# geopolars/geopolars

Measured on AMD Instinct MI355X. Metric: predicate evals/sec (10M pts x 1k polys point-in-polygon), higher is better.
Workload: dtype f64

## Files before the change

geopolars_amd/csrc/gpk_join.hip:

```cpp
#include <cstdlib>
#include <cstring>
#include <mutex>
#include <type_traits>

#include <rocprim/rocprim.hpp>

#include "gpk_device.h"
#include "gpk_index.h"
#include "gpk_candjoin.h"
#include "gpk_pip.h"
#include "gpk_scan.h"
#include "gpk_pipshared.h"

namespace gpk {

constexpr int PIP_BLOCK = 256;
constexpr int WR_BLOCK = 256;
constexpr int PIP_PPT = 2;
constexpr int PIP_TILE = PIP_BLOCK * PIP_PPT;
constexpr int PIP_GS = 8;
constexpr int PIP_OVF = 256;
constexpr int PIP_QCAP = PIP_BLOCK * PIP_PPT;
constexpr int PIP_SUPER_SHIFT = 6;
constexpr int PIP_WPT = 8;
// ... 1151 lines not shown
    for (int k = 0; k < PIP_WPT; ++k) {
        if (cnt[k] == 0) continue;
        const uint32_t l = left_base + (uint32_t)(i0 + k);
        if (c[k] != CODE_MULTI && (c[k] & CODE_POOL)) {
            const uint32_t at = c[k] & ~CODE_POOL;
            for (uint32_t t = 0; t < cnt[k]; ++t) emit(o++, make_uint2(l, multi_pool[at + 1 + t]));
            continue;
        }
        if (c[k] != CODE_MULTI) {
            emit(o++, make_uint2(l, c[k]));
            continue;
        }
        const double2 p = pts.xy[i0 + k];
        const GridParams g = *ix.grid;
        for_each_candidate(ix, g, p.x, p.y, [&](int j) {
            if (dev::valid_row(polys.validity, j) && dev::polygonal_hits_point<false>(polys, j, p.x, p.y)) emit(o++, make_uint2(l, (uint32_t)j));
        });
    }
    if (via_lds) {
        __syncthreads();
        const int n_out = (int)tot;
        for (int t = tid; t < n_out; t += WR_BLOCK)
            if (out_base + t < capacity) pairs[out_base + t] = s_pairs[t];
    }
}

constexpr size_t JOIN_STATS_WORDS = 8 + 8 * 8000;
static unsigned long long* g_join_stats = nullptr;
static bool g_join_stats_on = false;
unsigned long long* join_stats_buffer() { return g_join_stats_on ? g_join_stats : nullptr; }

static std::mutex g_fused_mu;
struct FusedDev {
    unsigned long long* slots = nullptr;
    unsigned long long tickets = 0;
    unsigned long long era = 0;
    int n = 0;
    hipEvent_t done = nullptr;
    hipStream_t last = nullptr;
    bool any = false;
};
static FusedDev g_fused[16];
static unsigned long long g_fused_epoch = 0;
struct FusedWords {
    unsigned long long *slots, *ticket, *lost;
    unsigned long long epoch, ticket_base;
};
static int32_t fused_launch_begin(hipStream_t s, int64_t n_words, int wgs, FusedWords* out) {
    int dev = 0;
    GPK_HIP(hipGetDevice(&dev));
    if (dev < 0 || dev >= 16) return fail(GPK_ERR_DEVICE, "spatial_join: device %d out of range", dev);
    if (n_words > (int64_t)0x7FFFFFF0ll) return fail(GPK_ERR_INVALID_ARGUMENT, "spatial_join: %lld epoch words", (long long)n_words);
    g_fused_mu.lock();
    FusedDev& f = g_fused[dev];
    auto bail = [&](hipError_t e) {
        g_fused_mu.unlock();
        return fail(GPK_ERR_DEVICE, "spatial_join: %s", hipGetErrorString(e));
    };
    if ((int64_t)f.n < n_words) {
        if (f.slots) {
            (void)hipDeviceSynchronize();
            (void)hipFree(f.slots);
            f.slots = nullptr;
        }
        const int want = n_words < 4096 ? 4096 : (int)n_words;
        const size_t bytes = sizeof(unsigned long long) * (size_t)(want + 2);
        hipError_t e = device_malloc((void**)&f.slots, bytes);
        if (e != hipSuccess) return bail(e);
        e = hipMemset(f.slots, 0, bytes);
        if (e != hipSuccess) return bail(e);
        f.n = want;
        f.tickets = 0;
        f.era = g_fused_epoch >> (64 - FUSED_TOTAL_BITS);
    }
    if (!f.done) {
        const hipError_t e = hipEventCreateWithFlags(&f.done, hipEventDisableTiming);
        if (e != hipSuccess) return bail(e);
    }
    if (f.any && f.last != s) {
        hipError_t e = hipEventRecord(f.done, f.last);
        if (e == hipSuccess) e = hipStreamWaitEvent(s, f.done, 0);
        if (e != hipSuccess) {
            (void)hipGetLastError();
            e = hipDeviceSynchronize();
            if (e != hipSuccess) return bail(e);
        }
    }
    ++g_fused_epoch;
    if ((g_fused_epoch & ((1ull << (64 - FUSED_TOTAL_BITS)) - 1ull)) == 0ull) ++g_fused_epoch;
    if ((g_fused_epoch >> (64 - FUSED_TOTAL_BITS)) != f.era) {
        const hipError_t e = hipMemsetAsync(f.slots, 0, sizeof(unsigned long long) * (size_t)(f.n + 1), s);
        if (e != hipSuccess) return bail(e);
        f.era = g_fused_epoch >> (64 - FUSED_TOTAL_BITS);
    }
    out->epoch = g_fused_epoch & ((1ull << (64 - FUSED_TOTAL_BITS)) - 1ull);
    out->slots = f.slots;
    out->lost = f.slots + f.n;
    out->ticket = f.slots + f.n + 1;
    out->ticket_base = f.tickets;
    f.tickets += (unsigned long long)wgs;
    return GPK_OK;
}
static void fused_launch_end(hipStream_t s, bool launched) {
    int dev = 0;
    (void)hipGetDevice(&dev);
    if (dev >= 0 && dev < 16) {
        g_fused[dev].last = s;
        g_fused[dev].any = true;
        if (!launched) g_fused[dev].n = 0;
    }
    g_fused_mu.unlock();
}

static int32_t pip_join_enqueue(const gpk_geoarray* left, const gpk_geoarray* right, const gpk_index* right_index, uint32_t left_row_base,
                                uint32_t* out_counts, uint32_t* out_pairs, int64_t pair_capacity, bool host_out,
                                unsigned long long* total_out, hipStream_t s, uint32_t** counts_dev_out, uint32_t** pairs_dev_out,
                                unsigned long long** grand_out) {
    const int64_t n = left->d.n_geoms;
    const bool lean = right_index->pip.R > 0 && right_index->pip_lean;
    static const bool no_flow = [] {
        const char* e = getenv("GPK_TILE_KERNEL");
        return e && !strcmp(e, "chain");
    }();
    PipView pvj = right_index->pip;
    pvj.slab_xy = right->d.xy;
    const bool chain = right_index->pip.R > 0 && right_index->pip.chain_xy != nullptr;
    const bool one_per_lane = !chain && !lean && right_index->pip.R > 0 && right_index->pip_list_heavy;
    const int flow_p = chain && !no_flow && right_index->pip.route != nullptr && right_index->pip.R <= PIP_ROUTE_RMAX
                           ? pip_flow_points_per_lane(n, right->d.n_geoms, right_index->pip.R, cu_count())
                           : 0;
    const bool flow = flow_p > 0;
    const int tile_points = flow ? 64 * flow_p : (chain ? 64 * CHAIN_PPT : (lean ? LEAN_TILE : (one_per_lane ? PIP_BLOCK : PIP_TILE)));
    const int64_t n_blocks = (n + tile_points - 1) / tile_points;
    const bool want_pairs = pair_capacity > 0;
    const size_t counts_bytes = sizeof(uint32_t) * (size_t)n;
    const size_t pairs_bytes = sizeof(uint32_t) * 2 * (size_t)pair_capacity;
    const int64_t n_super = (n_blocks >> PIP_SUPER_SHIFT) + 1;
    const int64_t n_wblocks = (n + PIP_WTILE - 1) / PIP_WTILE;
    const uint32_t multi_cap = chain ? 1024u : (uint32_t)(n < (int64_t)0x18000000 ? 2 * n + 1024 : (int64_t)0x30000000);
    int64_t flow_wgs = (int64_t)cu_count();
    {
        const int64_t want = (n_blocks + 15) / 16;
// ... 54 lines not shown
        hot.logR = 0;
        while ((1 << hot.logR) < pv.R) ++hot.logR;
        hot.rx0 = pv.rx0;
        hot.ry0 = pv.ry0;
        hot.inv_fw = pv.inv_fw;
        hot.inv_fh = pv.inv_fh;
        hot.cell = pv.cell;
        hot.half = reinterpret_cast<const HalfCell*>(pv.sub);
        hot.chain_xy = pv.chain_xy;
        hot.part_geom = pv.part_geom;
        hot.route = pv.route;
        hot.counts = counts_dev;
        hot.code = code;
        hot.block_tot = btot;
        hot.super_tot = stot;
        hot.stats = stats;
        hot.cold = cold;
        hot.stage = nullptr;
        hot.pool = reinterpret_cast<uint32_t*>(stage);
        hot.n_full_tiles = left->d.validity ? 0 : (int32_t)(n / tile_points);
        hot.inv_fw_s = pv.inv_fw * (double)PIP_SUB;
        hot.inv_fh_s = pv.inv_fh * (double)PIP_SUB;
        hot.sub_max = (double)(((uint32_t)PIP_SUB << hot.logR) - 1u);
    }
    if (flow) {
        const int64_t wgs = flow_wgs;
        FusedTail tail;
        memset(&tail, 0, sizeof tail);
        tail.pairs = (uint2*)pairs_dev;
        tail.capacity = pair_capacity;
        tail.grand = grand;
        tail.grand_host = total_out;
        tail.left_base = left_row_base;
        FusedWords fw;
        int32_t frc = fused_launch_begin(s, wgs, (int)wgs, &fw);
        if (frc != GPK_OK) return frc;
        tail.slots = fw.slots;
        tail.epoch = fw.epoch;
        tail.ticket = fw.ticket;
        tail.ticket_base = fw.ticket_base;
        tail.lost = fw.lost;
        frc = launch_pip_flow(hot, tail, (int)wgs, flow_p, s);
        fused_launch_end(s, frc == GPK_OK);
        if (frc != GPK_OK) return frc;
        *counts_dev_out = counts_dev;
        *pairs_dev_out = pairs_dev;
        *grand_out = grand;
        return GPK_OK;
    }
    if (chain)
        GPK_LAUNCH("gpk_pip_tile", pip_tile_chain_kernel, dim3((unsigned)((n_blocks + PIP_BLOCK / 64 - 1) / (PIP_BLOCK / 64))), dim3(PIP_BLOCK), 0, s, hot);
    else if (lean)
        GPK_LAUNCH("gpk_pip_tile", pip_tile_lean_kernel, dim3((unsigned)n_blocks), dim3(PIP_BLOCK), 0, s, left->d, right->d, right_index->v, pvj,
                 counts_dev, code, btot, stot, stats);
    else if (right_index->pip.R > 0)
        if (right_index->pip.sub2 && one_per_lane)
            GPK_LAUNCH("gpk_pip_tile", (pip_tile_kernel<true, true, 1>), dim3((unsigned)n_blocks), dim3(PIP_BLOCK), 0, s, left->d, right->d,
                     right_index->v, pvj, counts_dev, code, btot, stot, multi_pool, multi_cap, multi_top, stats);
        else if (right_index->pip.sub2)
            GPK_LAUNCH("gpk_pip_tile", (pip_tile_kernel<true, true>), dim3((unsigned)n_blocks), dim3(PIP_BLOCK), 0, s, left->d, right->d,
                     right_index->v, pvj, counts_dev, code, btot, stot, multi_pool, multi_cap, multi_top, stats);
        else if (one_per_lane)
            GPK_LAUNCH("gpk_pip_tile", (pip_tile_kernel<true, false, 1>), dim3((unsigned)n_blocks), dim3(PIP_BLOCK), 0, s, left->d, right->d,
                     right_index->v, pvj, counts_dev, code, btot, stot, multi_pool, multi_cap, multi_top, stats);
        else
            GPK_LAUNCH("gpk_pip_tile", (pip_tile_kernel<true, false>), dim3((unsigned)n_blocks), dim3(PIP_BLOCK), 0, s, left->d, right->d,
                     right_index->v, pvj, counts_dev, code, btot, stot, multi_pool, multi_cap, multi_top, stats);
    else
        GPK_LAUNCH("gpk_pip_tile_generic", (pip_tile_kernel<false, false>), dim3((unsigned)n_blocks), dim3(PIP_BLOCK), 0, s, left->d, right->d,
                 right_index->v, pvj, counts_dev, code, btot, stot, multi_pool, multi_cap, multi_top, stats);
    GPK_LAUNCH("gpk_pip_write", pip_write_kernel, dim3((unsigned)n_wblocks), dim3(WR_BLOCK), 0, s, left->d, right->d, right_index->v,
             code, btot, stot, (const uint32_t*)multi_pool, n_blocks, tile_points, left_row_base, (uint2*)pairs_dev, pair_capacity, grand, total_out);

    *counts_dev_out = counts_dev;
// ... 239 lines not shown
```

geopolars_amd/csrc/gpk_pipflow.hip:

```cpp
#include "gpk_pipshared.h"

namespace gpk {

constexpr int FLOW_P_MAX = 8;
constexpr int FLOW_BLOCK = 1024, FLOW_W = FLOW_BLOCK / 64;
constexpr int FLOW_ITEMS = 128;
constexpr int FLOW_PASS_AT = 40;
constexpr int FLOW_MAX_TILES = 1536;
constexpr int FLOW_ID_BITS = 22;
constexpr uint32_t FLOW_DEAD = 0xFFFFFFFFu;
constexpr uint32_t FLOW_MULTI = 0x80000000u;
constexpr uint32_t FLOW_PEND = FLOW_MULTI;
static_assert(64 * FLOW_P_MAX == 512, "an entry keeps the row within its tile in 9 bits");
static_assert(FLOW_MAX_TILES <= (1 << 14), "FlowItem::loc keeps the tile in 14 bits");

struct FlowItem {
    double px, py;
    uint32_t aux;
    uint32_t loc;
};
static_assert(sizeof(FlowItem) == 24, "list slot");

#ifdef GPK_TILE_TRACE
#define FLOW_STAMP(i)                                                                                                    \
    do {                                                                                                                 \
        if (h.stats && lane == 0 && wave % 5 == 0 && blockIdx.x < 900u) h.stats[8 + (blockIdx.x * 4 + wave / 5) * 16 + (i)] = wall_clock64(); \
    } while (0)
#if GPK_TILE_TRACE == 2
#define FLOW_PHASE(i)                                        \
    do {                                                     \
        asm volatile("s_waitcnt vmcnt(0) lgkmcnt(0)" ::: "memory"); \
        const unsigned long long _n = wall_clock64();        \
        g_phase[i] += _n - g_last;                           \
        g_last = _n;                                         \
    } while (0)
#define FLOW_PHASE_ARGS , unsigned long long (&g_phase)[6], unsigned long long& g_last
#define FLOW_PHASE_PASS , g_phase, g_last
#else
#define FLOW_PHASE(i) do {} while (0)
#define FLOW_PHASE_ARGS
#define FLOW_PHASE_PASS
#endif
#else
#define FLOW_STAMP(i) do {} while (0)
#define FLOW_PHASE(i) do {} while (0)
// ... 17 lines not shown
}

__device__ __forceinline__ void ring_edge_flat(double sx, double sy, double ex, double ey, double cx, double cy, int& wn, bool& on, bool& unsure) {
    const bool up = sy <= cy && ey >= cy, down = sy > cy && ey <= cy;
    const bool left = cx < fmin(sx, ex), within = !left && cx <= fmax(sx, ex);
    const double detleft = (sx - cx) * (ey - cy), detright = (sy - cy) * (ex - cx);
    const double det = detleft - detright;
    const double errbound = 3.3306690738754716e-16 * (fabs(detleft) + fabs(detright));
    const bool opposite = (detleft > 0.0 && detright <= 0.0) || (detleft < 0.0 && detright >= 0.0) || detleft == 0.0;
    const bool certain = opposite || fabs(det) >= errbound;
    const bool eval = (up || down) && within;
    unsure |= eval && !certain;
    on |= eval && certain && det == 0.0;
    wn += (up && ey != cy && (left || (within && det > 0.0))) ? 1 : 0;
    wn -= (down && (left || (within && det < 0.0))) ? 1 : 0;
}

__device__ __forceinline__ void flow_settle(const ChainHot& h, uint32_t* s_ttot, uint32_t t, uint32_t slot, uint32_t row, uint32_t li, uint32_t cnt,
                                            uint32_t first) {
    if (cnt == 0u) {
        h.pool[slot] = FLOW_DEAD;
        if (h.counts) h.counts[row] = 0u;
        atomicSub(&s_ttot[t], 1u);
    } else if (cnt == 1u) {
        h.pool[slot] = (first << 9) | li;
    } else {
        h.pool[slot] = FLOW_MULTI | (cnt << 9) | li;
        if (h.counts) h.counts[row] = cnt;
        atomicAdd(&s_ttot[t], cnt - 1u);
    }
}

template <int TS>
__device__ __forceinline__ void flow_exact_pass(const ChainHot& h, FlowItem* items, uint32_t& n_list, int lane, uint32_t* s_ttot, uint32_t tile0) {
    const uint32_t n = n_list < 64u ? n_list : 64u;
    wave_lds_fence();
    const bool act = (uint32_t)lane < n;
    double qx = 0.0, qy = 0.0;
    uint32_t hd = 0u, loc = 0u;
    if (act) {
        const FlowItem* it = items + lane;
        qx = it->px;
        qy = it->py;
        hd = it->aux;
        loc = it->loc;
    }
    const int count = (int)(hd & HCHAIN_COUNT_MASK);
    const double2* __restrict__ v = H_COLD(chain_xy) + (hd >> HCHAIN_START_SHIFT);
    const int i1 = count < 1 ? count : 1, i2 = count < 2 ? count : 2, i3 = count < 3 ? count : 3, i4 = count < 4 ? count : 4;
    double2 a0 = v[0], a1 = v[i1], a2 = v[i2], a3 = v[i3], a4 = v[i4];
    asm volatile("" : "+v"(a0.x), "+v"(a0.y), "+v"(a1.x), "+v"(a1.y), "+v"(a2.x), "+v"(a2.y), "+v"(a3.x), "+v"(a3.y), "+v"(a4.x), "+v"(a4.y));
    int wn = ((int)(hd << (28 - HCHAIN_BASE_SHIFT))) >> 28;
    bool unsure = false, on = false;
    ring_edge_flat(a0.x, a0.y, a1.x, a1.y, qx, qy, wn, on, unsure);
    ring_edge_flat(a1.x, a1.y, a2.x, a2.y, qx, qy, wn, on, unsure);
    ring_edge_flat(a2.x, a2.y, a3.x, a3.y, qx, qy, wn, on, unsure);
    ring_edge_flat(a3.x, a3.y, a4.x, a4.y, qx, qy, wn, on, unsure);
    if (count > 4) {
        double ax = a4.x, ay = a4.y;
        for (int j = 4; j < count; ++j) {
            const double2 b = v[j + 1];
            on |= dev::ring_edge_filtered(ax, ay, b.x, b.y, qx, qy, wn, unsure);
            ax = b.x;
            ay = b.y;
        }
    }
    const bool walk = act && (count == 0 || unsure);
    const bool inside = !on && wn != 0;
    const uint32_t t = loc >> 18, li = loc & 511u;
    const uint32_t slot = ((tile0 + t) << TS) + ((loc >> 9) & 511u), row = ((tile0 + t) << TS) + li;
    if (act && !walk && !inside) flow_settle(h, s_ttot, t, slot, row, li, 0u, 0u);
    unsigned long long wm = __ballot(walk);
#ifdef GPK_TILE_TRACE
    unsigned long long* const stats = nullptr;
#else
    unsigned long long* const stats = H_COLD(stats);
#endif
    if (stats) {
        const unsigned long long edges = wave_sum_u64((unsigned long long)(act ? count : 0));
        if (lane == 0) {
            atomicAdd(&stats[0], (unsigned long long)n);
            atomicAdd(&stats[1], edges);
            if (wm) atomicAdd(&stats[2], (unsigned long long)__popcll(wm));
        }
    }
    while (wm) {
        const int j = __builtin_ctzll(wm);
        wm &= wm - 1ull;
        const double x = __shfl(qx, j, 64), y = __shfl(qy, j, 64);
        const unsigned long long cf = chain_generic_row_first_call(H_COLD(cold), x, y, lane);
        if (lane == j) flow_settle(h, s_ttot, t, slot, row, li, (uint32_t)cf, (uint32_t)(cf >> 32));
    }
    n_list -= n;
    if (n_list) {
        FlowItem keep{};
        if ((uint32_t)lane < n_list) keep = items[64 + lane];
        wave_lds_fence();
        if ((uint32_t)lane < n_list) items[lane] = keep;
    }
    wave_lds_fence();
}

typedef uint32_t u32x4 __attribute__((ext_vector_type(4)));
// ... 2 lines not shown
                                                        uint32_t* s_ttot, uint32_t t, uint32_t tile, uint32_t n_ent, int lane, int ts) {
    asm volatile("s_waitcnt vmcnt(0)" ::: "memory");
    uint32_t* seg = pool + ((size_t)tile << ts);
    for (uint32_t i = 0; i < n_ent; i += 64u) {
        const uint32_t e = i + (uint32_t)lane < n_ent ? __hip_atomic_load(seg + i + lane, __ATOMIC_RELAXED, __HIP_MEMORY_SCOPE_AGENT) : 0u;
        unsigned long long pm = __ballot((e & ~511u) == FLOW_PEND);
        while (pm) {
            const int j = __builtin_ctzll(pm);
            pm &= pm - 1ull;
            const uint32_t li = (uint32_t)__shfl((int)e, j, 64) & 511u, row = (tile << ts) + li, slot = i + (uint32_t)j;
            const double2 q = pts_xy[row];
            const unsigned long long cf = chain_generic_row_first_call(cold, q.x, q.y, lane);
            const uint32_t cnt = (uint32_t)cf, first = (uint32_t)(cf >> 32);
            if (lane == 0) {
                if (stats) atomicAdd(&stats[2], 1ull);
                if (cnt == 0u) {
                    seg[slot] = FLOW_DEAD;
                    if (counts) counts[row] = 0u;
                    atomicSub(&s_ttot[t], 1u);
                } else if (cnt == 1u) {
                    seg[slot] = (first << 9) | li;
                } else {
                    seg[slot] = FLOW_MULTI | (cnt << 9) | li;
                    if (counts) counts[row] = cnt;
                    atomicAdd(&s_ttot[t], cnt - 1u);
                }
            }
        }
    }
}

template <bool SIMPLE, bool FULL, int P>
__device__ __forceinline__ void flow_tile(const ChainHot& h, const uint2* s_mask, const uint32_t* s_rec0, FlowItem* items, uint32_t& n_list, uint32_t t,
                                          uint32_t tile0, int lane, uint32_t* s_tcand, uint32_t* s_ttot FLOW_PHASE_ARGS) {
    constexpr int S = PIP_SUB, FLOW_TILE = 64 * P, TS = P == 8 ? 9 : (P == 4 ? 8 : (P == 2 ? 7 : 6));
    static_assert(P == 1 || P == 2 || P == 4 || P == 8, "tile sizes");
    static_assert(S == 8, "the sub-cell arithmetic below is written for 8 x 8 sub-cells");
    asm volatile("" : "+v"(lane));
    const uint32_t tile = tile0 + t;
    const int64_t base = (int64_t)tile * FLOW_TILE;
    const int64_t n_points = FULL ? 0 : H_COLD(n_points);
    const uint32_t rem = FULL ? (uint32_t)FLOW_TILE : (uint32_t)(n_points - base < (int64_t)FLOW_TILE ? n_points - base : (int64_t)FLOW_TILE);
    double px[P], py[P];
    {
        const double2* __restrict__ tile_xy = h.pts_xy + base;
        static_for<P>([&](auto K) {
            constexpr int k = decltype(K)::value;
            double2 v = make_double2(NAN, NAN);
            if (FULL || ((uint32_t)(k * 64 + lane) < rem && dev::valid_row(H_COLD(pts_validity), base + k * 64 + lane))) v = dev::load_stream(tile_xy + (k * 64 + lane));
            px[k] = v.x;
            py[k] = v.y;
        });
    }
    GPK_SCHED_FENCE();
    FLOW_PHASE(1);
    const int logR = h.logR;
    const uint32_t sub_max = ((uint32_t)S << logR) - 1u;
    uint32_t sidx4[(P + 3) / 4], gw[P];
    u32x4 rec[P];
    static_for<(P + 3) / 4>([&](auto J) { sidx4[decltype(J)::value] = 0u; });
    uint32_t sxs[P], sys_[P], r0s[P];
    uint2 ms[P];
    static_for<P>([&](auto K) {
        constexpr int k = decltype(K)::value;
        uint32_t sx = cvt_u32_sat((px[k] - h.rx0) * h.inv_fw_s), sy = cvt_u32_sat((py[k] - h.ry0) * h.inv_fh_s);
        sx = sx < sub_max ? sx : sub_max;
        sy = sy < sub_max ? sy : sub_max;
        const uint32_t at = ((sy >> 3) << (logR - 5)) + (sx >> 8);
        ms[k] = s_mask[at];
        r0s[k] = s_rec0[at];
        sxs[k] = sx;
        sys_[k] = sy;
// ... 82 lines not shown
    const bool live = e != FLOW_DEAD;
    const bool multi = live && (e & FLOW_MULTI) != 0u;
    const unsigned long long mm = __ballot(multi);
    if (__builtin_expect(mm == 0ull, 1)) {
        const unsigned long long m = __ballot(live);
        const uint32_t at = done + lanes_below(m);
        if (live && at < room) __builtin_nontemporal_store(((unsigned long long)(e >> 9) << 32) | (unsigned long long)(row0 + (e & 511u)), out64 + at);
        done += (uint32_t)__popcll(m);
        return;
    }
    const uint32_t n_out = !live ? 0u : (multi ? (e >> 9) & ((1u << FLOW_ID_BITS) - 1u) : 1u);
    uint32_t incl = n_out;
#pragma unroll
    for (int o = 1; o < 64; o <<= 1) {
        const uint32_t v = __shfl_up(incl, o, 64);
        if (lane >= o) incl += v;
    }
    const uint32_t at = done + incl - n_out;
    if (live && !multi && at < room) __builtin_nontemporal_store(((unsigned long long)(e >> 9) << 32) | (unsigned long long)(row0 + (e & 511u)), out64 + at);
    unsigned long long wm = mm;
    while (wm) {
        const int j = __builtin_ctzll(wm);
        wm &= wm - 1ull;
        const uint32_t lj = (uint32_t)__shfl((int)e, j, 64) & 511u, aj = (uint32_t)__shfl((int)at, j, 64);
        const double2 q = h.pts_xy[pt0 + lj];
        chain_generic_row_call(H_COLD(cold), q.x, q.y, lane, reinterpret_cast<uint2*>(out64 + aj), aj < room ? room - aj : 0u, row0 + lj);
    }
    done += (uint32_t)__shfl((int)incl, 63, 64);
}

template <bool SIMPLE, int P>
__global__ __launch_bounds__(FLOW_BLOCK) void pip_tile_flow_kernel(ChainHot h, FusedTail tail) {
    constexpr int WORDS = PIP_ROUTE_RMAX * PIP_ROUTE_RMAX / 32, W = FLOW_W, TS = P == 8 ? 9 : (P == 4 ? 8 : (P == 2 ? 7 : 6));
    __shared__ uint2 s_mask[WORDS];
    __shared__ uint32_t s_rec0[WORDS];
    __shared__ FlowItem s_items[W][FLOW_ITEMS];
    __shared__ uint32_t s_tcand[FLOW_MAX_TILES], s_ttot[FLOW_MAX_TILES];
    __shared__ uint32_t s_next, s_next2, s_wg, s_wgtot, s_gave_up;
    __shared__ unsigned long long s_part[W];
    const int lane = threadIdx.x & 63, wave = __builtin_amdgcn_readfirstlane(threadIdx.x >> 6);
    FLOW_STAMP(0);
    unsigned long long my_ticket = 0ull;
    if (threadIdx.x == 0) my_ticket = __hip_atomic_fetch_add(T_COLD(ticket), 1ull, __ATOMIC_RELAXED, __HIP_MEMORY_SCOPE_AGENT);
    {
        const int R = H_COLD(R), words = R * R / 32;
        const uint4* __restrict__ src = reinterpret_cast<const uint4*>(H_COLD(route));
        for (int i = threadIdx.x; i < words; i += FLOW_BLOCK) {
            const uint4 rw = src[i];
            s_mask[i] = make_uint2(rw.x, rw.y);
            s_rec0[i] = rw.z;
        }
    }
    FLOW_STAMP(1);
    if (threadIdx.x == 0) {
        s_wg = (uint32_t)(my_ticket - T_COLD(ticket_base));
        s_next = 0u;
        s_next2 = 0u;
        s_gave_up = 0u;
    }
    __syncthreads();
    const uint32_t wg = __builtin_amdgcn_readfirstlane(s_wg);
    const uint32_t T0 = (uint32_t)((int64_t)wg * H_COLD(n_tiles) / (int64_t)gridDim.x), T1 = (uint32_t)((int64_t)(wg + 1u) * H_COLD(n_tiles) / (int64_t)gridDim.x);
    const uint32_t nt = T1 - T0;
    const bool want_pairs = T_COLD(pairs) != nullptr;
    FLOW_STAMP(2);
    const uint32_t nf = (int64_t)T1 <= (int64_t)H_COLD(n_full_tiles) ? nt : ((int64_t)T0 >= (int64_t)H_COLD(n_full_tiles) ? 0u : (uint32_t)(H_COLD(n_full_tiles) - (int32_t)T0));
    uint32_t n_list = 0u;
#ifdef GPK_TILE_TRACE
    int n_mine = 0;
#if GPK_TILE_TRACE == 2
    unsigned long long g_phase[6] = {0ull, 0ull, 0ull, 0ull, 0ull, 0ull}, g_last = wall_clock64();
#endif
#endif
    auto draw = [&](uint32_t* counter) -> uint32_t {
        __builtin_amdgcn_wave_barrier();
        const uint32_t d = __hip_atomic_fetch_add(counter, 1u, __ATOMIC_RELAXED, __HIP_MEMORY_SCOPE_WORKGROUP);
        return __builtin_amdgcn_readfirstlane(d) >> 6;
    };
    {
        uint32_t t = draw(&s_next);
        while (t < nf) {
            const uint32_t tn = draw(&s_next);
            FLOW_PHASE(4);
            if (n_list >= (uint32_t)FLOW_PASS_AT) flow_exact_pass<TS>(h, s_items[wave], n_list, lane, s_ttot, T0);
            FLOW_PHASE(0);
            flow_tile<SIMPLE, true, P>(h, s_mask, s_rec0, s_items[wave], n_list, t, T0, lane, s_tcand, s_ttot FLOW_PHASE_PASS);
            t = tn;
#if defined(GPK_TILE_TRACE) && GPK_TILE_TRACE != 2
            if (n_mine < 6) FLOW_STAMP(3 + n_mine);
            ++n_mine;
#endif
        }
    }
    for (;;) {
        const uint32_t t = draw(&s_next2) + nf;
        if (t >= nt) break;
        if (n_list >= (uint32_t)FLOW_PASS_AT) flow_exact_pass<TS>(h, s_items[wave], n_list, lane, s_ttot, T0);
        flow_tile<SIMPLE, false, P>(h, s_mask, s_rec0, s_items[wave], n_list, t, T0, lane, s_tcand, s_ttot FLOW_PHASE_PASS);
    }
    while (n_list) flow_exact_pass<TS>(h, s_items[wave], n_list, lane, s_ttot, T0);
#if defined(GPK_TILE_TRACE) && GPK_TILE_TRACE == 2
    FLOW_PHASE(5);
    if (h.stats && lane == 0 && wave % 5 == 0 && blockIdx.x < 900u)
        for (int i = 0; i < 6; ++i) h.stats[8 + (blockIdx.x * 4 + wave / 5) * 16 + 3 + i] = g_phase[i];
#endif
    FLOW_STAMP(9);
    __syncthreads();
    FLOW_STAMP(10);
    constexpr int EM_C = P < 4 ? P : 4, EM_T = 24 / EM_C;
    uint32_t ent[EM_T][EM_C], cand[EM_T];
    auto em_request = [&](uint32_t first) {
        static_for<EM_T>([&](auto Rr) {
            constexpr int r = decltype(Rr)::value;
            const uint32_t et = first + (uint32_t)(r * W);
            cand[r] = et < nt && want_pairs ? s_tcand[et] : 0u;
            cand[r] = __builtin_amdgcn_readfirstlane(cand[r]);
            const uint32_t* seg = h.pool + ((size_t)(T0 + et) << TS);
            static_for<EM_C>([&](auto Cc) {
                constexpr int c = decltype(Cc)::value;
                ent[r][c] = FLOW_DEAD;
                if ((uint32_t)(c * 64 + lane) < cand[r]) ent[r][c] = seg[c * 64 + lane];
            });
        });
    };
    em_request((uint32_t)wave);
    if (wave == 0) {
        uint32_t carry = 0u;
        for (uint32_t c0 = 0; c0 < nt; c0 += 64u) {
            const uint32_t v = c0 + (uint32_t)lane < nt ? s_ttot[c0 + lane] : 0u;
            uint32_t incl = v;
#pragma unroll
            for (int o = 1; o < 64; o <<= 1) {
                const uint32_t a = __shfl_up(incl, o, 64);
                if (lane >= o) incl += a;
            }
            if (c0 + (uint32_t)lane < nt) s_ttot[c0 + lane] = carry + incl - v;
            carry += (uint32_t)__shfl((int)incl, 63, 64);
        }
        if (lane == 0) s_wgtot = carry;
    }
    __syncthreads();
    const unsigned long long wg_tot = (unsigned long long)s_wgtot;
    const unsigned long long epoch = T_COLD(epoch);
    unsigned long long* const slots = T_COLD(slots);
    if (threadIdx.x == 0) __hip_atomic_store(&slots[wg], (epoch << FUSED_TOTAL_BITS) | wg_tot, __ATOMIC_RELAXED, __HIP_MEMORY_SCOPE_AGENT);
    unsigned long long acc = 0;
    bool gave_up = false;
    for (unsigned b = threadIdx.x; b < wg; b += FLOW_BLOCK) {
        unsigned long long v;
        uint32_t spins = 0;
        while (((v = __hip_atomic_load(&slots[b], __ATOMIC_RELAXED, __HIP_MEMORY_SCOPE_AGENT)) >> FUSED_TOTAL_BITS) != epoch) {
            __builtin_amdgcn_s_sleep(8);
            if (++spins > FUSED_SPIN_LIMIT) {
                gave_up = true;
                break;
            }
        }
        acc += v & ((1ull << FUSED_TOTAL_BITS) - 1ull);
    }
    if (gave_up) __hip_atomic_store(&s_gave_up, 1u, __ATOMIC_RELAXED, __HIP_MEMORY_SCOPE_WORKGROUP);
    acc = wave_sum_u64(acc);
    if (lane == 0) s_part[wave] = acc;
    __syncthreads();
    const bool lost = s_gave_up != 0u;
    unsigned long long base_off = 0;
#pragma unroll
    for (int w = 0; w < W; ++w) base_off += s_part[w];
    if ((wg == gridDim.x - 1 || lost) && threadIdx.x == 0) {
        unsigned long long* const lostp = T_COLD(lost);
        if (lost) __hip_atomic_store(lostp, epoch, __ATOMIC_RELAXED, __HIP_MEMORY_SCOPE_AGENT);
        const bool any_lost = lost || __hip_atomic_load(lostp, __ATOMIC_RELAXED, __HIP_MEMORY_SCOPE_AGENT) == epoch;
        unsigned long long* const grand = T_COLD(grand);
        unsigned long long* const grand_host = T_COLD(grand_host);
        *grand = any_lost ? FUSED_LOST : base_off + wg_tot;
        if (grand_host) *grand_host = any_lost ? FUSED_LOST : base_off + wg_tot;
    }
    FLOW_STAMP(11);
    if (!want_pairs || lost) return;
    unsigned long long* const pairs64 = reinterpret_cast<unsigned long long*>(T_COLD(pairs));
    const int64_t capacity = T_COLD(capacity);
    const uint32_t left_base = T_COLD(left_base);
    for (uint32_t first = (uint32_t)wave; first < nt; first += (uint32_t)(EM_T * W)) {
        if (first != (uint32_t)wave) em_request(first);
        static_for<EM_T>([&](auto Rr) {
            constexpr int r = decltype(Rr)::value;
            const uint32_t et = first + (uint32_t)(r * W);
            if (cand[r]) {
                const unsigned long long off = base_off + (unsigned long long)s_ttot[et];
                unsigned long long* const out64 = pairs64 + off;
                const int64_t left = capacity - (int64_t)off;
                const uint32_t room = left <= 0 ? 0u : (left > (int64_t)0xFFFFFFFFll ? 0xFFFFFFFFu : (uint32_t)left);
                const uint32_t pt0 = (T0 + et) << TS, row0 = pt0 + left_base;
                uint32_t done = 0u;
                static_for<EM_C>([&](auto Cc) {
                    constexpr int c = decltype(Cc)::value;
                    if ((uint32_t)(c * 64) < cand[r]) flow_emit_chunk(h, ent[r][c], row0, pt0, out64, room, done, lane);
                });
                if (EM_C * 64 < 64 * P) {
                    const uint32_t* seg = h.pool + ((size_t)(T0 + et) << TS);
                    for (uint32_t i = (uint32_t)(EM_C * 64); i < cand[r]; i += 64u) {
                        const uint32_t e = i + (uint32_t)lane < cand[r] ? seg[i + lane] : FLOW_DEAD;
                        flow_emit_chunk(h, e, row0, pt0, out64, room, done, lane);
                    }
                }
            }
        });
    }
    FLOW_STAMP(12);
}

int pip_flow_points_per_lane(int64_t n_left_rows, int64_t n_right_geoms, int32_t R, int wgs) {
    if (R < 32 || R > PIP_ROUTE_RMAX || wgs < 1) return 0;
    if (n_right_geoms >= (int64_t)((1u << FLOW_ID_BITS) - 1u)) return 0;
    if (n_left_rows >= (int64_t)0xFFFFFE00ll) return 0;
    static const int forced = [] {
        const char* e = getenv("GPK_FLOW_P");
        return e ? atoi(e) : 0;
    }();
    const int64_t waves = (int64_t)wgs * FLOW_W;
    for (int p = FLOW_P_MAX; p >= 1; p >>= 1) {
        const int64_t n_tiles = (n_left_rows + 64 * p - 1) / (64 * p);
        if ((n_tiles + wgs - 1) / wgs > (int64_t)FLOW_MAX_TILES) return p == FLOW_P_MAX ? 0 : 2 * p;
        if (forced ? p == forced : (n_tiles >= waves || p == 1)) return p;
    }
    return 1;
}
size_t pip_flow_pool_bytes(int64_t n_left_rows) { return sizeof(uint32_t) * (size_t)((n_left_rows + 511) / 512) * 512u; }

template <int P>
static int32_t launch_pip_flow_p(const ChainHot& hot, const FusedTail& tail, int wgs, hipStream_t s) {
    if (hot.part_geom == nullptr && hot.polys_validity == nullptr)
        GPK_LAUNCH("gpk_pip_tile", (pip_tile_flow_kernel<true, P>), dim3((unsigned)wgs), dim3(FLOW_BLOCK), 0, s, hot, tail);
// ... 16 lines not shown
```

geopolars_amd/csrc/gpk_pipshared.h:

```cpp
#pragma once

#include <type_traits>

#include "gpk_device.h"
#include "gpk_index.h"

namespace gpk {

constexpr uint32_t CODE_NONE = 0xFFFFFFFFu, CODE_MULTI = 0xFFFFFFFEu;
constexpr uint32_t CODE_POOL = 0x80000000u;

#define GPK_SCHED_FENCE() __builtin_amdgcn_sched_barrier(0)
template <int N, typename F>
__device__ __forceinline__ void static_for(F&& f) {
    if constexpr (N > 0) {
        static_for<N - 1>(f);
        f(std::integral_constant<int, N - 1>{});
    }
}

struct ChainHot {
    const double2* pts_xy;
    const uint8_t* pts_validity;
    int64_t n_points, n_tiles;
// ... 69 lines not shown
                    pos = dev::POS_OUTSIDE;
            }
            hit = r1 > r0 && pos == dev::POS_INSIDE;
        }
        if (hit) {
            if (cnt == 0) *first = (uint32_t)j;
            if (emit != nullptr && lane == 0 && cnt < emit_room) emit[cnt] = make_uint2(l, (uint32_t)j);
            ++cnt;
        }
    }
    return cnt;
}

__device__ __forceinline__ uint32_t lanes_below(unsigned long long m) {
    return __builtin_amdgcn_mbcnt_hi((uint32_t)(m >> 32), __builtin_amdgcn_mbcnt_lo((uint32_t)m, 0u));
}
template <typename T>
__device__ __forceinline__ T kernel_arg_at(uint32_t offset) {
    const char __attribute__((address_space(4)))* ka = (const char __attribute__((address_space(4)))*)__builtin_amdgcn_kernarg_segment_ptr();
    asm volatile("" : "+s"(ka));
    return *(const T __attribute__((address_space(4)))*)(ka + offset);
}

static __device__ __noinline__ uint32_t chain_generic_row_call(const ChainCold* cold, double px, double py, int lane, uint2* emit, uint32_t emit_room, uint32_t l) {
    uint32_t first;
    return chain_generic_row<false>(cold, px, py, lane, &first, emit, emit_room, l);
}
static __device__ __noinline__ unsigned long long chain_generic_row_first_call(const ChainCold* cold, double px, double py, int lane) {
    uint32_t first;
    const uint32_t cnt = chain_generic_row<false>(cold, px, py, lane, &first);
    return ((unsigned long long)first << 32) | cnt;
}

struct FusedTail {
    uint2* pairs;
    int64_t capacity;
    unsigned long long* slots;
    unsigned long long epoch;
    unsigned long long* grand;
    unsigned long long* grand_host;
    uint32_t left_base, pad;
    unsigned long long* ticket;
    unsigned long long ticket_base;
    unsigned long long* lost;
};

constexpr int FUSED_TOTAL_BITS = 40;
constexpr uint32_t FUSED_SPIN_LIMIT = 1u << 22;
constexpr unsigned long long FUSED_LOST = ~0ull;

__device__ __forceinline__ unsigned long long wave_sum_u64(unsigned long long v) {
#pragma unroll
    for (int o = 32; o > 0; o >>= 1) v += __shfl_xor(v, o, 64);
    return v;
}

int pip_flow_points_per_lane(int64_t n_left_rows, int64_t n_right_geoms, int32_t R, int wgs);
size_t pip_flow_pool_bytes(int64_t n_left_rows);
int32_t launch_pip_flow(const ChainHot& hot, const FusedTail& tail, int wgs, int points_per_lane, hipStream_t s);

}
```

Measured before the change: 116700 billion.

## Deal tiles to work-groups dynamically in chunks and rework the fused offset scan

Replaces the static per-work-group tile range (set by a ticket index) with a global atomic dealer. Each work-group grabs chunks of 16 tiles on demand, and waves resolve tile indices through an LDS chunk table. The cross-work-group prefix sum over per-slot totals is replaced by per-chunk totals and a settled counter that every group waits on, after which each group scans all chunk totals to find its output offsets. The aim is better load balance across work-groups with uneven polygon cost. In exchange it adds atomics, spin waits, and a redundant full scan of chunk totals in every group.

```diff
diff --git a/geopolars_amd/csrc/gpk_join.hip b/geopolars_amd/csrc/gpk_join.hip
--- a/geopolars_amd/csrc/gpk_join.hip
+++ b/geopolars_amd/csrc/gpk_join.hip
@@ -1207,46 +1207,41 @@
 
 static std::mutex g_fused_mu;
 struct FusedDev {
-    unsigned long long* slots = nullptr;
-    unsigned long long tickets = 0;
-    unsigned long long era = 0;
-    int n = 0;
+    unsigned long long* words = nullptr;
+    unsigned long long deal = 0;
+    unsigned long long settled = 0;
+    bool stale = false;
     hipEvent_t done = nullptr;
     hipStream_t last = nullptr;
     bool any = false;
 };
 static FusedDev g_fused[16];
 static unsigned long long g_fused_epoch = 0;
-struct FusedWords {
-    unsigned long long *slots, *ticket, *lost;
-    unsigned long long epoch, ticket_base;
-};
-static int32_t fused_launch_begin(hipStream_t s, int64_t n_words, int wgs, FusedWords* out) {
+constexpr int FUSED_WORDS = 48;
+static int32_t fused_launch_begin(hipStream_t s, int64_t n_tiles, int wgs, FusedTail* tail) {
     int dev = 0;
     GPK_HIP(hipGetDevice(&dev));
     if (dev < 0 || dev >= 16) return fail(GPK_ERR_DEVICE, "spatial_join: device %d out of range", dev);
-    if (n_words > (int64_t)0x7FFFFFF0ll) return fail(GPK_ERR_INVALID_ARGUMENT, "spatial_join: %lld epoch words", (long long)n_words);
+    if (n_tiles > (int64_t)0x7FFFFFF0ll) return fail(GPK_ERR_INVALID_ARGUMENT, "spatial_join: %lld tiles", (long long)n_tiles);
     g_fused_mu.lock();
     FusedDev& f = g_fused[dev];
     auto bail = [&](hipError_t e) {
         g_fused_mu.unlock();
         return fail(GPK_ERR_DEVICE, "spatial_join: %s", hipGetErrorString(e));
     };
-    if ((int64_t)f.n < n_words) {
-        if (f.slots) {
-            (void)hipDeviceSynchronize();
-            (void)hipFree(f.slots);
-            f.slots = nullptr;
-        }
-        const int want = n_words < 4096 ? 4096 : (int)n_words;
-        const size_t bytes = sizeof(unsigned long long) * (size_t)(want + 2);
-        hipError_t e = device_malloc((void**)&f.slots, bytes);
+    if (f.words && f.stale) {
+        (void)hipDeviceSynchronize();
+        (void)hipFree(f.words);
+        f.words = nullptr;
+    }
+    if (!f.words) {
+        const size_t bytes = sizeof(unsigned long long) * (size_t)FUSED_WORDS;
+        hipError_t e = device_malloc((void**)&f.words, bytes);
         if (e != hipSuccess) return bail(e);
-        e = hipMemset(f.slots, 0, bytes);
+        e = hipMemset(f.words, 0, bytes);
         if (e != hipSuccess) return bail(e);
-        f.n = want;
-        f.tickets = 0;
-        f.era = g_fused_epoch >> (64 - FUSED_TOTAL_BITS);
+        f.deal = f.settled = 0;
+        f.stale = false;
     }
     if (!f.done) {
         const hipError_t e = hipEventCreateWithFlags(&f.done, hipEventDisableTiming);
@@ -1261,19 +1256,15 @@
             if (e != hipSuccess) return bail(e);
         }
     }
-    ++g_fused_epoch;
-    if ((g_fused_epoch & ((1ull << (64 - FUSED_TOTAL_BITS)) - 1ull)) == 0ull) ++g_fused_epoch;
-    if ((g_fused_epoch >> (64 - FUSED_TOTAL_BITS)) != f.era) {
-        const hipError_t e = hipMemsetAsync(f.slots, 0, sizeof(unsigned long long) * (size_t)(f.n + 1), s);
-        if (e != hipSuccess) return bail(e);
-        f.era = g_fused_epoch >> (64 - FUSED_TOTAL_BITS);
-    }
-    out->epoch = g_fused_epoch & ((1ull << (64 - FUSED_TOTAL_BITS)) - 1ull);
-    out->slots = f.slots;
-    out->lost = f.slots + f.n;
-    out->ticket = f.slots + f.n + 1;
-    out->ticket_base = f.tickets;
-    f.tickets += (unsigned long long)wgs;
+    tail->epoch = ++g_fused_epoch;
+    tail->lost = f.words;
+    tail->deal = f.words + 16;
+    tail->deal_base = f.deal;
+    f.deal += (unsigned long long)FLOW_CHUNK * (unsigned long long)((n_tiles + FLOW_CHUNK - 1) / FLOW_CHUNK + wgs);
+    tail->deal_end = f.deal;
+    tail->settled = f.words + 32;
+    tail->settled_base = f.settled;
+    f.settled += ((unsigned long long)wgs << FUSED_TILE_BITS) + (unsigned long long)n_tiles;
     return GPK_OK;
 }
 static void fused_launch_end(hipStream_t s, bool launched) {
@@ -1282,7 +1273,7 @@
     if (dev >= 0 && dev < 16) {
         g_fused[dev].last = s;
         g_fused[dev].any = true;
-        if (!launched) g_fused[dev].n = 0;
+        if (!launched) g_fused[dev].stale = true;
     }
     g_fused_mu.unlock();
 }
@@ -1403,14 +1394,8 @@
         tail.grand = grand;
         tail.grand_host = total_out;
         tail.left_base = left_row_base;
-        FusedWords fw;
-        int32_t frc = fused_launch_begin(s, wgs, (int)wgs, &fw);
+        int32_t frc = fused_launch_begin(s, n_blocks, (int)wgs, &tail);
         if (frc != GPK_OK) return frc;
-        tail.slots = fw.slots;
-        tail.epoch = fw.epoch;
-        tail.ticket = fw.ticket;
-        tail.ticket_base = fw.ticket_base;
-        tail.lost = fw.lost;
         frc = launch_pip_flow(hot, tail, (int)wgs, flow_p, s);
         fused_launch_end(s, frc == GPK_OK);
         if (frc != GPK_OK) return frc;
diff --git a/geopolars_amd/csrc/gpk_pipflow.hip b/geopolars_amd/csrc/gpk_pipflow.hip
--- a/geopolars_amd/csrc/gpk_pipflow.hip
+++ b/geopolars_amd/csrc/gpk_pipflow.hip
@@ -11,6 +11,12 @@
 constexpr uint32_t FLOW_DEAD = 0xFFFFFFFFu;
 constexpr uint32_t FLOW_MULTI = 0x80000000u;
 constexpr uint32_t FLOW_PEND = FLOW_MULTI;
+constexpr int FLOW_MAX_CHUNKS = FLOW_MAX_TILES / FLOW_CHUNK;
+constexpr uint32_t FLOW_NONE = 0xFFFFFFFFu;
+constexpr uint32_t FLOW_WAIT = 0xFFFFFFFFu;
+constexpr uint32_t FLOW_DEALT_OUT = 0xFFFFFFF0u;
+static_assert(FLOW_W == FLOW_CHUNK, "a chunk is a tile for each wave of the work-group");
+static_assert(FLOW_MAX_TILES % FLOW_CHUNK == 0, "whole chunks");
 static_assert(64 * FLOW_P_MAX == 512, "an entry keeps the row within its tile in 9 bits");
 static_assert(FLOW_MAX_TILES <= (1 << 14), "FlowItem::loc keeps the tile in 14 bits");
 
@@ -94,7 +100,7 @@
 }
 
 template <int TS>
-__device__ __forceinline__ void flow_exact_pass(const ChainHot& h, FlowItem* items, uint32_t& n_list, int lane, uint32_t* s_ttot, uint32_t tile0) {
+__device__ __forceinline__ void flow_exact_pass(const ChainHot& h, FlowItem* items, uint32_t& n_list, int lane, uint32_t* s_ttot, const uint32_t* s_chunk) {
     const uint32_t n = n_list < 64u ? n_list : 64u;
     wave_lds_fence();
     const bool act = (uint32_t)lane < n;
@@ -130,7 +136,8 @@
     const bool walk = act && (count == 0 || unsure);
     const bool inside = !on && wn != 0;
     const uint32_t t = loc >> 18, li = loc & 511u;
-    const uint32_t slot = ((tile0 + t) << TS) + ((loc >> 9) & 511u), row = ((tile0 + t) << TS) + li;
+    const uint32_t tile = s_chunk[t / FLOW_CHUNK] + t % FLOW_CHUNK;
+    const uint32_t slot = (tile << TS) + ((loc >> 9) & 511u), row = (tile << TS) + li;
     if (act && !walk && !inside) flow_settle(h, s_ttot, t, slot, row, li, 0u, 0u);
     unsigned long long wm = __ballot(walk);
 #ifdef GPK_TILE_TRACE
@@ -199,12 +206,11 @@
 
 template <bool SIMPLE, bool FULL, int P>
 __device__ __forceinline__ void flow_tile(const ChainHot& h, const uint2* s_mask, const uint32_t* s_rec0, FlowItem* items, uint32_t& n_list, uint32_t t,
-                                          uint32_t tile0, int lane, uint32_t* s_tcand, uint32_t* s_ttot FLOW_PHASE_ARGS) {
+                                          uint32_t tile, int lane, uint32_t* s_tcand, uint32_t* s_ttot FLOW_PHASE_ARGS) {
     constexpr int S = PIP_SUB, FLOW_TILE = 64 * P, TS = P == 8 ? 9 : (P == 4 ? 8 : (P == 2 ? 7 : 6));
     static_assert(P == 1 || P == 2 || P == 4 || P == 8, "tile sizes");
     static_assert(S == 8, "the sub-cell arithmetic below is written for 8 x 8 sub-cells");
     asm volatile("" : "+v"(lane));
-    const uint32_t tile = tile0 + t;
     const int64_t base = (int64_t)tile * FLOW_TILE;
     const int64_t n_points = FULL ? 0 : H_COLD(n_points);
     const uint32_t rem = FULL ? (uint32_t)FLOW_TILE : (uint32_t)(n_points - base < (int64_t)FLOW_TILE ? n_points - base : (int64_t)FLOW_TILE);
@@ -353,16 +359,23 @@
 template <bool SIMPLE, int P>
 __global__ __launch_bounds__(FLOW_BLOCK) void pip_tile_flow_kernel(ChainHot h, FusedTail tail) {
     constexpr int WORDS = PIP_ROUTE_RMAX * PIP_ROUTE_RMAX / 32, W = FLOW_W, TS = P == 8 ? 9 : (P == 4 ? 8 : (P == 2 ? 7 : 6));
+    constexpr uint32_t CH = (uint32_t)FLOW_CHUNK;
     __shared__ uint2 s_mask[WORDS];
     __shared__ uint32_t s_rec0[WORDS];
     __shared__ FlowItem s_items[W][FLOW_ITEMS];
     __shared__ uint32_t s_tcand[FLOW_MAX_TILES], s_ttot[FLOW_MAX_TILES];
-    __shared__ uint32_t s_next, s_next2, s_wg, s_wgtot, s_gave_up;
-    __shared__ unsigned long long s_part[W];
+    __shared__ uint32_t s_chunk[FLOW_MAX_CHUNKS];
+    __shared__ unsigned long long s_cpre[FLOW_MAX_CHUNKS];
+    __shared__ unsigned long long s_wsum[W];
+    __shared__ uint32_t s_next, s_nt, s_gave_up;
     const int lane = threadIdx.x & 63, wave = __builtin_amdgcn_readfirstlane(threadIdx.x >> 6);
     FLOW_STAMP(0);
-    unsigned long long my_ticket = 0ull;
-    if (threadIdx.x == 0) my_ticket = __hip_atomic_fetch_add(T_COLD(ticket), 1ull, __ATOMIC_RELAXED, __HIP_MEMORY_SCOPE_AGENT);
+    auto deal = [&]() -> uint32_t {
+        const unsigned long long d = __hip_atomic_fetch_add(T_COLD(deal), (unsigned long long)CH, __ATOMIC_RELAXED, __HIP_MEMORY_SCOPE_AGENT) - T_COLD(deal_base);
+        return d < (unsigned long long)FLOW_DEALT_OUT ? (uint32_t)d : FLOW_DEALT_OUT;
+    };
+    uint32_t chunk0 = FLOW_DEALT_OUT;
+    if (threadIdx.x == 0) chunk0 = deal();
     {
         const int R = H_COLD(R), words = R * R / 32;
         const uint4* __restrict__ src = reinterpret_cast<const uint4*>(H_COLD(route));
@@ -373,19 +386,17 @@
         }
     }
     FLOW_STAMP(1);
+    const uint32_t n_tiles = (uint32_t)H_COLD(n_tiles);
+    if (threadIdx.x > 0 && threadIdx.x < (unsigned)FLOW_MAX_CHUNKS) s_chunk[threadIdx.x] = FLOW_WAIT;
     if (threadIdx.x == 0) {
-        s_wg = (uint32_t)(my_ticket - T_COLD(ticket_base));
+        s_chunk[0] = chunk0;
+        s_nt = chunk0 < n_tiles ? (n_tiles - chunk0 < CH ? n_tiles - chunk0 : CH) : 0u;
         s_next = 0u;
-        s_next2 = 0u;
         s_gave_up = 0u;
     }
     __syncthreads();
-    const uint32_t wg = __builtin_amdgcn_readfirstlane(s_wg);
-    const uint32_t T0 = (uint32_t)((int64_t)wg * H_COLD(n_tiles) / (int64_t)gridDim.x), T1 = (uint32_t)((int64_t)(wg + 1u) * H_COLD(n_tiles) / (int64_t)gridDim.x);
-    const uint32_t nt = T1 - T0;
     const bool want_pairs = T_COLD(pairs) != nullptr;
     FLOW_STAMP(2);
-    const uint32_t nf = (int64_t)T1 <= (int64_t)H_COLD(n_full_tiles) ? nt : ((int64_t)T0 >= (int64_t)H_COLD(n_full_tiles) ? 0u : (uint32_t)(H_COLD(n_full_tiles) - (int32_t)T0));
     uint32_t n_list = 0u;
 #ifdef GPK_TILE_TRACE
     int n_mine = 0;
@@ -393,33 +404,53 @@
     unsigned long long g_phase[6] = {0ull, 0ull, 0ull, 0ull, 0ull, 0ull}, g_last = wall_clock64();
 #endif
 #endif
-    auto draw = [&](uint32_t* counter) -> uint32_t {
+    auto draw = [&]() -> uint32_t {
         __builtin_amdgcn_wave_barrier();
-        const uint32_t d = __hip_atomic_fetch_add(counter, 1u, __ATOMIC_RELAXED, __HIP_MEMORY_SCOPE_WORKGROUP);
+        const uint32_t d = __hip_atomic_fetch_add(&s_next, 1u, __ATOMIC_RELAXED, __HIP_MEMORY_SCOPE_WORKGROUP);
         return __builtin_amdgcn_readfirstlane(d) >> 6;
     };
+    auto resolve = [&](uint32_t t) -> uint32_t {
+        if (t >= (uint32_t)FLOW_MAX_TILES) return FLOW_NONE;
+        const uint32_t c = t / CH;
+        uint32_t b;
+        while ((b = __hip_atomic_load(&s_chunk[c], __ATOMIC_RELAXED, __HIP_MEMORY_SCOPE_WORKGROUP)) == FLOW_WAIT) __builtin_amdgcn_s_sleep(2);
+        b = __builtin_amdgcn_readfirstlane(b);
+        const uint32_t nt_col = (uint32_t)H_COLD(n_tiles);
+        if (t % CH == 0u && c + 1u < (uint32_t)FLOW_MAX_CHUNKS && lane == 0) {
+            uint32_t nb = FLOW_DEALT_OUT;
+            if (b < nt_col) {
+                nb = deal();
+                if (nb < nt_col) atomicAdd(&s_nt, nt_col - nb < CH ? nt_col - nb : CH);
+            }
+            __hip_atomic_store(&s_chunk[c + 1u], nb, __ATOMIC_RELAXED, __HIP_MEMORY_SCOPE_WORKGROUP);
+        }
+        const uint32_t g = b + t % CH;
+        return g < nt_col ? g : FLOW_NONE;
+    };
     {
-        uint32_t t = draw(&s_next);
-        while (t < nf) {
-            const uint32_t tn = draw(&s_next);
+        uint32_t t = draw(), g = resolve(t);
+        while (g < (uint32_t)H_COLD(n_full_tiles)) {
+            const uint32_t tn = draw();
             FLOW_PHASE(4);
-            if (n_list >= (uint32_t)FLOW_PASS_AT) flow_exact_pass<TS>(h, s_items[wave], n_list, lane, s_ttot, T0);
+            if (n_list >= (uint32_t)FLOW_PASS_AT) flow_exact_pass<TS>(h, s_items[wave], n_list, lane, s_ttot, s_chunk);
             FLOW_PHASE(0);
-            flow_tile<SIMPLE, true, P>(h, s_mask, s_rec0, s_items[wave], n_list, t, T0, lane, s_tcand, s_ttot FLOW_PHASE_PASS);
+            flow_tile<SIMPLE, true, P>(h, s_mask, s_rec0, s_items[wave], n_list, t, g, lane, s_tcand, s_ttot FLOW_PHASE_PASS);
             t = tn;
+            g = resolve(t);
 #if defined(GPK_TILE_TRACE) && GPK_TILE_TRACE != 2
             if (n_mine < 6) FLOW_STAMP(3 + n_mine);
             ++n_mine;
 #endif
         }
-    }
-    for (;;) {
-        const uint32_t t = draw(&s_next2) + nf;
-        if (t >= nt) break;
-        if (n_list >= (uint32_t)FLOW_PASS_AT) flow_exact_pass<TS>(h, s_items[wave], n_list, lane, s_ttot, T0);
-        flow_tile<SIMPLE, false, P>(h, s_mask, s_rec0, s_items[wave], n_list, t, T0, lane, s_tcand, s_ttot FLOW_PHASE_PASS);
-    }
-    while (n_list) flow_exact_pass<TS>(h, s_items[wave], n_list, lane, s_ttot, T0);
+        while (g != FLOW_NONE) {
+            const uint32_t tn = draw();
+            if (n_list >= (uint32_t)FLOW_PASS_AT) flow_exact_pass<TS>(h, s_items[wave], n_list, lane, s_ttot, s_chunk);
+            flow_tile<SIMPLE, false, P>(h, s_mask, s_rec0, s_items[wave], n_list, t, g, lane, s_tcand, s_ttot FLOW_PHASE_PASS);
+            t = tn;
+            g = resolve(t);
+        }
+    }
+    while (n_list) flow_exact_pass<TS>(h, s_items[wave], n_list, lane, s_ttot, s_chunk);
 #if defined(GPK_TILE_TRACE) && GPK_TILE_TRACE == 2
     FLOW_PHASE(5);
     if (h.stats && lane == 0 && wave % 5 == 0 && blockIdx.x < 900u)
@@ -428,6 +459,8 @@
     FLOW_STAMP(9);
     __syncthreads();
     FLOW_STAMP(10);
+    const uint32_t nt = __builtin_amdgcn_readfirstlane(s_nt);
+    const uint32_t n_ch = (nt + CH - 1u) / CH;
     constexpr int EM_C = P < 4 ? P : 4, EM_T = 24 / EM_C;
     uint32_t ent[EM_T][EM_C], cand[EM_T];
     auto em_request = [&](uint32_t first) {
@@ -436,7 +469,8 @@
             const uint32_t et = first + (uint32_t)(r * W);
             cand[r] = et < nt && want_pairs ? s_tcand[et] : 0u;
             cand[r] = __builtin_amdgcn_readfirstlane(cand[r]);
-            const uint32_t* seg = h.pool + ((size_t)(T0 + et) << TS);
+            const uint32_t tile = et < nt ? __builtin_amdgcn_readfirstlane(s_chunk[et / CH]) + et % CH : 0u;
+            const uint32_t* seg = h.pool + ((size_t)tile << TS);
             static_for<EM_C>([&](auto Cc) {
                 constexpr int c = decltype(Cc)::value;
                 ent[r][c] = FLOW_DEAD;
@@ -445,6 +479,7 @@
         });
     };
     em_request((uint32_t)wave);
+    const unsigned long long settled_base = T_COLD(settled_base);
     if (wave == 0) {
         uint32_t carry = 0u;
         for (uint32_t c0 = 0; c0 < nt; c0 += 64u) {
@@ -458,43 +493,79 @@
             if (c0 + (uint32_t)lane < nt) s_ttot[c0 + lane] = carry + incl - v;
             carry += (uint32_t)__shfl((int)incl, 63, 64);
         }
-        if (lane == 0) s_wgtot = carry;
-    }
-    __syncthreads();
-    const unsigned long long wg_tot = (unsigned long long)s_wgtot;
-    const unsigned long long epoch = T_COLD(epoch);
-    unsigned long long* const slots = T_COLD(slots);
-    if (threadIdx.x == 0) __hip_atomic_store(&slots[wg], (epoch << FUSED_TOTAL_BITS) | wg_tot, __ATOMIC_RELAXED, __HIP_MEMORY_SCOPE_AGENT);
-    unsigned long long acc = 0;
-    bool gave_up = false;
-    for (unsigned b = threadIdx.x; b < wg; b += FLOW_BLOCK) {
-        unsigned long long v;
-        uint32_t spins = 0;
-        while (((v = __hip_atomic_load(&slots[b], __ATOMIC_RELAXED, __HIP_MEMORY_SCOPE_AGENT)) >> FUSED_TOTAL_BITS) != epoch) {
-            __builtin_amdgcn_s_sleep(8);
-            if (++spins > FUSED_SPIN_LIMIT) {
-                gave_up = true;
-                break;
-            }
-        }
-        acc += v & ((1ull << FUSED_TOTAL_BITS) - 1ull);
-    }
-    if (gave_up) __hip_atomic_store(&s_gave_up, 1u, __ATOMIC_RELAXED, __HIP_MEMORY_SCOPE_WORKGROUP);
-    acc = wave_sum_u64(acc);
-    if (lane == 0) s_part[wave] = acc;
+        wave_lds_fence();
+        unsigned long long* const chunk_tot = h.block_tot;
+        unsigned long long seen = 0ull;
+        for (uint32_t c = (uint32_t)lane; c < n_ch; c += 64u) {
+            const uint32_t end = (c + 1u) * CH < nt ? s_ttot[(c + 1u) * CH] : carry;
+            seen |= __hip_atomic_exchange(&chunk_tot[s_chunk[c] / CH], (unsigned long long)(end - s_ttot[c * CH]), __ATOMIC_RELAXED, __HIP_MEMORY_SCOPE_AGENT);
+        }
+        asm volatile("s_waitcnt vmcnt(0)" : "+v"(seen)::"memory");
+        __builtin_amdgcn_wave_barrier();
+        if (lane == 0) {
+            unsigned long long* const settled = T_COLD(settled);
+            const unsigned long long before =
+                __hip_atomic_fetch_add(settled, (1ull << FUSED_TILE_BITS) | (unsigned long long)nt, __ATOMIC_RELAXED, __HIP_MEMORY_SCOPE_AGENT) - settled_base;
+            if ((before >> FUSED_TILE_BITS) == (unsigned long long)(gridDim.x - 1u)) __hip_atomic_store(T_COLD(deal), T_COLD(deal_end), __ATOMIC_RELAXED, __HIP_MEMORY_SCOPE_AGENT);
+            if (nt) {
+                uint32_t spins = 0;
+                while (((__hip_atomic_load(settled, __ATOMIC_RELAXED, __HIP_MEMORY_SCOPE_AGENT) - settled_base) & ((1ull << FUSED_TILE_BITS) - 1ull)) < (unsigned long long)n_tiles) {
+                    __builtin_amdgcn_s_sleep(8);
+                    if (++spins > FUSED_SPIN_LIMIT) {
+                        __hip_atomic_store(&s_gave_up, 1u, __ATOMIC_RELAXED, __HIP_MEMORY_SCOPE_WORKGROUP);
+                        break;
+                    }
+                }
+            }
+        }
+    }
+    if (nt == 0u) return;
     __syncthreads();
     const bool lost = s_gave_up != 0u;
-    unsigned long long base_off = 0;
+    unsigned long long launch_tot = 0ull;
+    if (!lost) {
+        unsigned long long* const s_texcl = reinterpret_cast<unsigned long long*>(&s_items[0][0]);
+        static_assert(sizeof(FlowItem) * W * FLOW_ITEMS >= sizeof(unsigned long long) * FLOW_BLOCK, "scan scratch");
+        const unsigned long long* const chunk_tot = h.block_tot;
+        const uint32_t n_chunks = (n_tiles + CH - 1u) / CH, R = (n_chunks + (uint32_t)FLOW_BLOCK - 1u) / (uint32_t)FLOW_BLOCK;
+        const uint32_t j0 = threadIdx.x * R;
+        const bool mine = threadIdx.x < n_ch;
+        const uint32_t k = mine ? s_chunk[threadIdx.x] / CH : 0u, o = k / R;
+        auto ld = [&](uint32_t j, bool on) { return on ? __hip_atomic_load(&chunk_tot[j], __ATOMIC_RELAXED, __HIP_MEMORY_SCOPE_AGENT) : 0ull; };
+        unsigned long long tsum = 0ull, part = 0ull;
+        for (uint32_t i = 0; i < R; i += 2u) {
+            const unsigned long long a0 = ld(j0 + i, j0 + i < n_chunks), a1 = ld(j0 + i + 1u, i + 1u < R && j0 + i + 1u < n_chunks);
+            const unsigned long long b0 = ld(o * R + i, mine && o * R + i < k), b1 = ld(o * R + i + 1u, mine && o * R + i + 1u < k);
+            tsum += a0 + a1;
+            part += b0 + b1;
+        }
+        unsigned long long incl = tsum;
 #pragma unroll
-    for (int w = 0; w < W; ++w) base_off += s_part[w];
-    if ((wg == gridDim.x - 1 || lost) && threadIdx.x == 0) {
+        for (int d = 1; d < 64; d <<= 1) {
+            const unsigned long long a = __shfl_up(incl, d, 64);
+            if (lane >= d) incl += a;
+        }
+        s_texcl[threadIdx.x] = incl - tsum;
+        if (lane == 63) s_wsum[wave] = incl;
+        __syncthreads();
+        if (mine) {
+            unsigned long long pre = part + s_texcl[o];
+            for (uint32_t w = 0; w < o / 64u; ++w) pre += s_wsum[w];
+            s_cpre[threadIdx.x] = pre;
+        }
+#pragma unroll
+        for (int w = 0; w < W; ++w) launch_tot += s_wsum[w];
+        __syncthreads();
+    }
+    if (threadIdx.x == 0 && (lost || s_chunk[n_ch - 1u] / CH == (n_tiles - 1u) / CH)) {
         unsigned long long* const lostp = T_COLD(lost);
+        const unsigned long long epoch = T_COLD(epoch);
         if (lost) __hip_atomic_store(lostp, epoch, __ATOMIC_RELAXED, __HIP_MEMORY_SCOPE_AGENT);
         const bool any_lost = lost || __hip_atomic_load(lostp, __ATOMIC_RELAXED, __HIP_MEMORY_SCOPE_AGENT) == epoch;
         unsigned long long* const grand = T_COLD(grand);
         unsigned long long* const grand_host = T_COLD(grand_host);
-        *grand = any_lost ? FUSED_LOST : base_off + wg_tot;
-        if (grand_host) *grand_host = any_lost ? FUSED_LOST : base_off + wg_tot;
+        *grand = any_lost ? FUSED_LOST : launch_tot;
+        if (grand_host) *grand_host = any_lost ? FUSED_LOST : launch_tot;
     }
     FLOW_STAMP(11);
     if (!want_pairs || lost) return;
@@ -507,18 +578,20 @@
             constexpr int r = decltype(Rr)::value;
             const uint32_t et = first + (uint32_t)(r * W);
             if (cand[r]) {
-                const unsigned long long off = base_off + (unsigned long long)s_ttot[et];
+                const uint32_t ec = et / CH;
+                const unsigned long long off = s_cpre[ec] + (unsigned long long)(uint32_t)(s_ttot[et] - s_ttot[ec * CH]);
                 unsigned long long* const out64 = pairs64 + off;
                 const int64_t left = capacity - (int64_t)off;
                 const uint32_t room = left <= 0 ? 0u : (left > (int64_t)0xFFFFFFFFll ? 0xFFFFFFFFu : (uint32_t)left);
-                const uint32_t pt0 = (T0 + et) << TS, row0 = pt0 + left_base;
+                const uint32_t tile = __builtin_amdgcn_readfirstlane(s_chunk[ec]) + et % CH;
+                const uint32_t pt0 = tile << TS, row0 = pt0 + left_base;
                 uint32_t done = 0u;
                 static_for<EM_C>([&](auto Cc) {
                     constexpr int c = decltype(Cc)::value;
                     if ((uint32_t)(c * 64) < cand[r]) flow_emit_chunk(h, ent[r][c], row0, pt0, out64, room, done, lane);
                 });
                 if (EM_C * 64 < 64 * P) {
-                    const uint32_t* seg = h.pool + ((size_t)(T0 + et) << TS);
+                    const uint32_t* seg = h.pool + ((size_t)tile << TS);
                     for (uint32_t i = (uint32_t)(EM_C * 64); i < cand[r]; i += 64u) {
                         const uint32_t e = i + (uint32_t)lane < cand[r] ? seg[i + lane] : FLOW_DEAD;
                         flow_emit_chunk(h, e, row0, pt0, out64, room, done, lane);
diff --git a/geopolars_amd/csrc/gpk_pipshared.h b/geopolars_amd/csrc/gpk_pipshared.h
--- a/geopolars_amd/csrc/gpk_pipshared.h
+++ b/geopolars_amd/csrc/gpk_pipshared.h
@@ -125,20 +125,23 @@
     return ((unsigned long long)first << 32) | cnt;
 }
 
+constexpr int FLOW_CHUNK = 16;
+constexpr int FUSED_TILE_BITS = 40;
 struct FusedTail {
     uint2* pairs;
     int64_t capacity;
-    unsigned long long* slots;
-    unsigned long long epoch;
+    unsigned long long* deal;
+    unsigned long long deal_base;
+    unsigned long long deal_end;
+    unsigned long long* settled;
+    unsigned long long settled_base;
     unsigned long long* grand;
     unsigned long long* grand_host;
     uint32_t left_base, pad;
-    unsigned long long* ticket;
-    unsigned long long ticket_base;
     unsigned long long* lost;
+    unsigned long long epoch;
 };
 
-constexpr int FUSED_TOTAL_BITS = 40;
 constexpr uint32_t FUSED_SPIN_LIMIT = 1u << 22;
 constexpr unsigned long long FUSED_LOST = ~0ull;
 
```

New measurement: 100300 billion. 0.86x the previous value.
